# haesungpyun/seoul_tourism_recommendation_NGCF

Measured on AMD Instinct MI355X. Metric: NGCF 3-layer forward: propagated edges/sec + achieved HBM GB/s, d=128, higher is better.
Workload: dtype f32

## Files before the change

include/ngcf_hip.h:

```cpp
#ifndef NGCF_HIP_H
#define NGCF_HIP_H

#include <stdint.h>

#ifdef __cplusplus
extern "C" {
#endif

#define NGCF_OK            0
#define NGCF_ERR_ARG       1
#define NGCF_ERR_HIP       2
#define NGCF_ERR_INDEX     3
#define NGCF_ERR_WORKSPACE 4

typedef struct ngcf_csr ngcf_csr_t;

const char *ngcf_last_error(void);
const char *ngcf_target_arch(void);
#define NGCF_ABI_VERSION 11
int ngcf_version(void);

int ngcf_options_from_env(void);
int ngcf_set_option(const char *name, int64_t value);

int ngcf_prof_enable(int on);
int ngcf_prof_collect(int64_t *n_launches, double *total_ms);

int ngcf_csr_from_coo(const int64_t *rows, const int64_t *cols, const float *vals, int64_t nnz,
                      int64_t n_rows, int64_t n_cols, ngcf_csr_t **out, void *stream);
int ngcf_csr_from_arrays(const int64_t *rowptr, const int32_t *colidx, const float *vals,
                         int64_t n_rows, int64_t n_cols, int64_t nnz, ngcf_csr_t **out, void *stream);
int ngcf_csr_plan(ngcf_csr_t *csr, int32_t seg_len, void *stream);
int ngcf_csr_set_mode(ngcf_csr_t *csr, int mode, void *stream);
int ngcf_csr_filter(const ngcf_csr_t *src, const uint8_t *keep, const int32_t *map, int64_t nnz_kept, ngcf_csr_t **dst,
                    void *stream);
const int32_t *ngcf_csr_filter_pos(const ngcf_csr_t *dst);
int ngcf_csr_filter_remap(const ngcf_csr_t *dst_t, const uint8_t *keep, const int32_t *map, int64_t n_src_entries,
                          const int32_t *pos_l, int32_t *map_out, void *stream);
void ngcf_csr_free(ngcf_csr_t *csr);
int64_t ngcf_csr_nnz(const ngcf_csr_t *csr);
int64_t ngcf_csr_n_rows(const ngcf_csr_t *csr);
int64_t ngcf_csr_n_cols(const ngcf_csr_t *csr);
int64_t ngcf_csr_n_segments(const ngcf_csr_t *csr);
int64_t ngcf_csr_max_row_len(const ngcf_csr_t *csr);
int64_t ngcf_csr_swept_rows(const ngcf_csr_t *csr);
const int64_t *ngcf_csr_rowptr(const ngcf_csr_t *csr);
const int32_t *ngcf_csr_colidx(const ngcf_csr_t *csr);
const float *ngcf_csr_vals(const ngcf_csr_t *csr);

int64_t ngcf_spmm_workspace_bytes(const ngcf_csr_t *csr, int d);
int64_t ngcf_layer_workspace_bytes(const ngcf_csr_t *csr, int d_in, int d_out);

int ngcf_spmm_csr_f32(const ngcf_csr_t *csr, const float *E, int64_t ldE, int d, float *LE,
                      int64_t ldLE, void *workspace, int64_t workspace_bytes, void *stream);

int ngcf_spmm_product_width(const ngcf_csr_t *csr, const float *E, int64_t ldE, int d);

int ngcf_spmm_csr_dropout_f32(const ngcf_csr_t *csr, const float *E, int64_t ldE, int d, float *LE, int64_t ldLE,
                              float drop_p, const uint64_t *seeds, int n_seeds, int transposed,
                              void *workspace, int64_t workspace_bytes, void *stream);

int ngcf_layer_fused_f32(const ngcf_csr_t *csr, const float *E_gather, int64_t ldEg,
                         const float *E_self, int64_t ldEs, int d_in,
                         const float *W1, const float *b1, const float *W2, const float *b2, int d_out,
                         float leaky_slope, float drop_p, uint64_t drop_seed,
                         const float *drop_mask, int64_t ld_mask,
                         float *carry, int64_t ldc, float *norm, int64_t ldn,
                         void *workspace, int64_t workspace_bytes, void *stream);

int64_t ngcf_dense_workspace_bytes(int d_in, int d_out);
int ngcf_layer_dense_f32(const float *LE, int64_t ldLE, const float *E_self, int64_t ldEs,
                         int64_t n_rows, int d_in,
                         const float *W1, const float *b1, const float *W2, const float *b2, int d_out,
                         float leaky_slope, float drop_p, uint64_t drop_seed,
                         const float *drop_mask, int64_t ld_mask,
                         float *carry, int64_t ldc, float *norm, int64_t ldn,
                         void *workspace, int64_t workspace_bytes, void *stream);

// ... 125 lines not shown
```

seoul_tourism_recommendation_ngcf_amd/_lib.py:

```python
from __future__ import annotations

import ctypes as C
import os
import sys

import torch

from . import _build

OK, ERR_ARG, ERR_HIP, ERR_INDEX, ERR_WORKSPACE = 0, 1, 2, 3, 4
ABI_VERSION = 11

_vp, _i64, _i32, _f32, _u64 = C.c_void_p, C.c_int64, C.c_int32, C.c_float, C.c_uint64

PROTOTYPES = {
    "ngcf_last_error": (C.c_char_p, []),
    "ngcf_target_arch": (C.c_char_p, []),
    "ngcf_version": (C.c_int, []),
    "ngcf_options_from_env": (C.c_int, []),
    "ngcf_set_option": (C.c_int, [C.c_char_p, _i64]),
    "ngcf_prof_enable": (C.c_int, [C.c_int]),
    "ngcf_prof_collect": (C.c_int, [C.POINTER(_i64), C.POINTER(C.c_double)]),
    "ngcf_csr_from_coo": (C.c_int, [_vp, _vp, _vp, _i64, _i64, _i64, C.POINTER(_vp), _vp]),
    "ngcf_csr_from_arrays": (C.c_int, [_vp, _vp, _vp, _i64, _i64, _i64, C.POINTER(_vp), _vp]),
    "ngcf_csr_plan": (C.c_int, [_vp, _i32, _vp]),
    "ngcf_csr_set_mode": (C.c_int, [_vp, C.c_int, _vp]),
    "ngcf_csr_filter": (C.c_int, [_vp, _vp, _vp, _i64, C.POINTER(_vp), _vp]),
    "ngcf_csr_filter_pos": (_vp, [_vp]),
    "ngcf_csr_filter_remap": (C.c_int, [_vp, _vp, _vp, _i64, _vp, _vp, _vp]),
    "ngcf_csr_free": (None, [_vp]),
    "ngcf_csr_nnz": (_i64, [_vp]),
    "ngcf_csr_n_rows": (_i64, [_vp]),
    "ngcf_csr_n_cols": (_i64, [_vp]),
    "ngcf_csr_n_segments": (_i64, [_vp]),
    "ngcf_csr_max_row_len": (_i64, [_vp]),
    "ngcf_csr_swept_rows": (_i64, [_vp]),
    "ngcf_csr_rowptr": (_vp, [_vp]),
    "ngcf_csr_colidx": (_vp, [_vp]),
    "ngcf_csr_vals": (_vp, [_vp]),
    "ngcf_spmm_workspace_bytes": (_i64, [_vp, C.c_int]),
    "ngcf_layer_workspace_bytes": (_i64, [_vp, C.c_int, C.c_int]),
    "ngcf_dense_workspace_bytes": (_i64, [C.c_int, C.c_int]),
    "ngcf_spmm_product_width": (C.c_int, [_vp, _vp, _i64, C.c_int]),
    "ngcf_spmm_csr_f32": (C.c_int, [_vp, _vp, _i64, C.c_int, _vp, _i64, _vp, _i64, _vp]),
    "ngcf_spmm_csr_dropout_f32": (C.c_int, [_vp, _vp, _i64, C.c_int, _vp, _i64, _f32, C.POINTER(_u64), C.c_int, C.c_int,
                                            _vp, _i64, _vp]),
    "ngcf_layer_fused_f32": (C.c_int, [_vp, _vp, _i64, _vp, _i64, C.c_int, _vp, _vp, _vp, _vp, C.c_int,
                                       _f32, _f32, _u64, _vp, _i64, _vp, _i64, _vp, _i64, _vp, _i64, _vp]),
    "ngcf_layer_dense_f32": (C.c_int, [_vp, _i64, _vp, _i64, _i64, C.c_int, _vp, _vp, _vp, _vp, C.c_int,
                                       _f32, _f32, _u64, _vp, _i64, _vp, _i64, _vp, _i64, _vp, _i64, _vp]),
    "ngcf_copy_rows_f32": (C.c_int, [_vp, _i64, _vp, _i64, _i64, C.c_int, _vp]),
    "ngcf_copy_rows2_f32": (C.c_int, [_vp, _i64, _vp, _i64, _vp, _i64, _i64, C.c_int, _vp]),
    "ngcf_copy_rows_indexed_f32": (C.c_int, [_vp, _i64, _vp, _i64, _vp, _i64, _i64, C.c_int, _vp]),
    "ngcf_feature_inject_f32": (C.c_int, [_vp, _i64, _i64, C.c_int, C.POINTER(_vp), C.POINTER(_vp),
                                          C.POINTER(_i64), C.c_int, _vp, _i64, C.c_double, _vp, _vp, _vp]),
    "ngcf_seeds_advance": (C.c_int, [_vp, C.c_int, _vp]),
    "ngcf_gather_rows_f32": (C.c_int, [_vp, _i64, C.c_int, _vp, _i64, _i64, _i64, _vp, _i64, _vp, _vp]),
    "ngcf_gather_rows3_f32": (C.c_int, [_vp, _i64, C.c_int] + [_vp, _i64, _i64, _i64, _vp] * 3 + [_i64, _vp, _vp]),
    "ngcf_bpr_workspace_bytes": (_i64, [_i64]),
    "ngcf_bpr_fused_f32": (C.c_int, [_vp, _i64, _vp, _i64, _vp, _i64, C.c_int, _f32, _f32, _vp, _vp, _i64, _vp]),
    "ngcf_bpr_backward_f32": (C.c_int, [_vp, _i64, _vp, _i64, _vp, _i64, C.c_int, _f32, _f32, _vp, _vp, _vp, _vp, _vp]),
    "ngcf_rows_sort_unique": (C.c_int, [_vp, _i64, _i64, _vp, _vp, _vp, _vp, _vp]),
    "ngcf_segment_sum_rows_f32": (C.c_int, [_vp, _i64, C.c_int, _vp, _vp, _i64, _vp, _vp, _vp, _i64, _i64, _vp]),
    "ngcf_layer_bwd_pre_f32": (C.c_int, [_vp, _i64, _vp, _i64, _vp, _i64, _i64, C.c_int, _f32, _f32, _u64, _vp, _i64,
                                         _vp, _vp, _i64, _vp]),
    "ngcf_spmm_t_rows_f32": (C.c_int, [_vp, _vp, _vp, _i64, C.c_int, _vp, _i64, _vp, _i64, _f32, C.POINTER(_u64), C.c_int, _vp, _i64, _vp]),
    "ngcf_layer_bwd_input_workspace_bytes": (_i64, [C.c_int]),
    "ngcf_layer_bwd_input_f32": (C.c_int, [_vp, _i64, _i64, C.c_int, _vp, _vp, C.c_int, _vp, _i64, _vp, _i64, _vp, _i64, _vp, _i64,
                                           _vp, _i64, _vp]),
# ... 105 lines not shown
```

seoul_tourism_recommendation_ngcf_amd/csrc/common.h:

```cpp
#ifndef NGCF_COMMON_H
#define NGCF_COMMON_H

#include <hip/hip_runtime.h>

#include <algorithm>
#include <cstdarg>
#include <cstdint>
#include <cstdio>
#include <cstdlib>
#include <cstring>
#include <numeric>
#include <thread>
#include <vector>

#include "../../include/ngcf_hip.h"

inline thread_local char g_err[512] = "";

inline int fail(int code, const char *fmt, ...)
{
    va_list ap;
    va_start(ap, fmt);
    vsnprintf(g_err, sizeof(g_err), fmt, ap);
    va_end(ap);
// ... 90 lines not shown
    float *vals = nullptr;
    bool owns = false;
    int64_t cap = 0, pos_len = 0;
    int32_t *pos = nullptr;
    int32_t *scan_blk = nullptr;
    bool borrows_plan = false;
    const struct ngcf_csr *filter_src = nullptr;
    int32_t seg_len = 0;
    int64_t n_seg = 0, n_heavy = 0;
    int32_t *seg_row = nullptr;
    int64_t *seg_begin = nullptr;
    int32_t *heavy_row = nullptr;
    int64_t *heavy_seg_ptr = nullptr;
    struct RowGroup {
        int64_t begin, end;
        bool sliceable;
        int32_t col_lo, col_hi;
        bool lds_table = false;
    };
    std::vector<RowGroup> groups;
    int mode = 0;
    struct SegSet {
        int64_t n_seg = 0, n_heavy = 0;
        int32_t *seg_row = nullptr;
        int64_t *seg_begin = nullptr;
        int32_t *heavy_row = nullptr;
        int64_t *heavy_seg_ptr = nullptr;
    };
    struct Swept {
        struct Part {
            int64_t row_lo = 0, row_hi = 0;
            int waves = 0, rows_per_wave = 0;
            int lpe = 16;
            int32_t n_rowpass = 0, n_win = 0, win_cols = 0, col_lo = 0, col_hi = 0;
            int64_t n_slots = 0, n_partial = 0, n_heavy = 0, partial_base = 0;
            int64_t *tptr = nullptr;
            int32_t *e_pack = nullptr;
            float *e_val = nullptr;
            int32_t *dst = nullptr;
            int32_t *prow = nullptr;
            int32_t *heavy_row = nullptr;
            int64_t *heavy_seg_ptr = nullptr;
        };
        std::vector<Part> parts;
        std::vector<char> group_swept;
        SegSet out;
        int64_t n_partial = 0;
        uint32_t *barrier = nullptr;
        mutable hipStream_t barrier_owner[4] = {nullptr, nullptr, nullptr, nullptr};
        mutable int barrier_used = 0;
        int built_mode = 0;
        int lpe = 16;
    } swept;
};


static const int32_t kLdsTableRows = 512;
static const int32_t kDefaultSegLen = 2048;
static inline int32_t default_seg_len(int64_t nnz)
{
    int32_t s = 64;
    while (s < kDefaultSegLen && (int64_t)s * 4096 < nnz) s *= 2;
    return s;
}

void free_swept(ngcf_csr *c);
int build_swept_plan(ngcf_csr *c, hipStream_t stream);
bool swept_usable(const ngcf_csr *c, int64_t ldE, int d);
void prof_mark(hipStream_t stream, int which);

__host__ __device__ inline uint64_t fmix64(uint64_t x)
{
    x ^= x >> 33;
    x *= 0xff51afd7ed558ccdULL;
    x ^= x >> 33;
    x *= 0xc4ceb9fe1a85ec53ULL;
    x ^= x >> 33;
    return x;
}
__device__ inline uint32_t mix32(uint64_t x) { return (uint32_t)fmix64(x); }

__device__ __forceinline__ uint32_t msg_drop_thr(float drop_p)
{
    return drop_p > 0.f ? (uint32_t)((double)drop_p * 4294967296.0) : 0u;
}
// ... 35 lines not shown
    r.s1 = dr.n > 1 ? resolve_seed(dr.seed[1]) : 0;
    r.s2 = dr.n > 2 ? resolve_seed(dr.seed[2]) : 0;
    r.s3 = dr.n > 3 ? resolve_seed(dr.seed[3]) : 0;
    return r;
}

__device__ inline bool edge_keep(const EdgeDropR &dr, int64_t row, int64_t col)
{
    const uint64_t i = (uint64_t)(dr.transposed ? col : row), j = (uint64_t)(dr.transposed ? row : col);
    const uint64_t e = ((i << 32) | (j & 0xffffffffull)) * 0x9E3779B97F4A7C15ULL;
    bool keep = true;
    if (dr.n > 0) keep = mix32(dr.s0 ^ e) >= dr.thr;
    if (dr.n > 1) keep = keep && mix32(dr.s1 ^ e) >= dr.thr;
    if (dr.n > 2) keep = keep && mix32(dr.s2 ^ e) >= dr.thr;
    if (dr.n > 3) keep = keep && mix32(dr.s3 ^ e) >= dr.thr;
    return keep;
}


int spmm_dispatch(const ngcf_csr *c, const float *E, int64_t ldE, int d, float *out, int64_t ldo, void *workspace,
                  int64_t workspace_bytes, hipStream_t stream, const EdgeDrop &dr = EdgeDrop{0, 0, {0, 0, 0, 0}, 0});
int launch_swept(const ngcf_csr *c, const float *E, int64_t ldE, int d, float *out, int64_t ldo, float *partial, int dp,
                 hipStream_t stream, const EdgeDrop &dr);

template <int U> __device__ inline int row_bcast(int x)
{
    return __builtin_amdgcn_update_dpp(0, x, 0x150 + U, 0xf, 0xf, false);
}
template <int U> __device__ inline float row_bcast(float x)
{
    return __int_as_float(__builtin_amdgcn_update_dpp(0, __float_as_int(x), 0x150 + U, 0xf, 0xf, false));
}

template <int VEC> struct VecT;
template <> struct VecT<4> { using type = float4; };
template <> struct VecT<2> { using type = float2; };
template <> struct VecT<1> { using type = float; };

__device__ inline float4 vfma(float s, float4 x, float4 a)
{
    a.x = fmaf(s, x.x, a.x);
    a.y = fmaf(s, x.y, a.y);
    a.z = fmaf(s, x.z, a.z);
    a.w = fmaf(s, x.w, a.w);
    return a;
}
__device__ inline float vfma(float s, float x, float a) { return fmaf(s, x, a); }
__device__ inline float2 vfma(float s, float2 x, float2 a)
{
    a.x = fmaf(s, x.x, a.x);
    a.y = fmaf(s, x.y, a.y);
    return a;
}
__device__ inline float2 vadd(float2 a, float2 b) { return make_float2(a.x + b.x, a.y + b.y); }
__device__ inline float2 vshfl_xor(float2 a, int m)
{
    a.x = __shfl_xor(a.x, m);
    a.y = __shfl_xor(a.y, m);
    return a;
}
__device__ inline float4 vsel(bool p, float4 a, float4 b) { return p ? a : b; }
__device__ inline float vsel(bool p, float a, float b) { return p ? a : b; }
__device__ inline float4 vzero4() { return make_float4(0.f, 0.f, 0.f, 0.f); }
template <int VEC> __device__ inline typename VecT<VEC>::type vzero();
template <> __device__ inline float4 vzero<4>() { return vzero4(); }
template <> __device__ inline float vzero<1>() { return 0.f; }
// ... 40 lines not shown
```

seoul_tourism_recommendation_ngcf_amd/csrc/csr.hip:

```cpp
#include "common.h"

extern "C" const char *ngcf_last_error(void) { return g_err; }
extern "C" const char *ngcf_target_arch(void) { return "gfx950"; }
extern "C" int ngcf_version(void) { return NGCF_ABI_VERSION; }

NgcfOptions g_opts;

namespace {
struct OptField {
    const char *name;
    int NgcfOptions::*i;
    int64_t NgcfOptions::*l;
};
const OptField kOptFields[] = {
    {"no_fork", &NgcfOptions::no_fork, nullptr},
    {"no_slicing", &NgcfOptions::no_slicing, nullptr},
    {"no_ldstab", &NgcfOptions::no_ldstab, nullptr},
    {"no_panel_split", &NgcfOptions::no_panel_split, nullptr},
    {"no_tail_table", &NgcfOptions::no_tail_table, nullptr},
    {"no_pad_product", &NgcfOptions::no_pad_product, nullptr},
    {"fork_min", nullptr, &NgcfOptions::fork_min},
    {"dense_direct", &NgcfOptions::dense_direct, nullptr},
    {"dense_resident", &NgcfOptions::dense_resident, nullptr},
    {"dense_resident_min_rows", &NgcfOptions::dense_resident_min_rows, nullptr},
// ... 72 lines not shown
    c->seg_row = nullptr;
    c->seg_begin = nullptr;
    c->heavy_row = nullptr;
    c->heavy_seg_ptr = nullptr;
    c->n_seg = c->n_heavy = 0;
}

extern "C" void ngcf_csr_free(ngcf_csr_t *c)
{
    if (!c) return;
    free_plan(c);
    free_swept(c);
    if (c->owns) {
        if (c->rowptr) (void)hipFree(c->rowptr);
        if (c->colidx) (void)hipFree(c->colidx);
        if (c->vals) (void)hipFree(c->vals);
    }
    if (c->pos) (void)hipFree(c->pos);
    if (c->scan_blk) (void)hipFree(c->scan_blk);
    delete c;
}

extern "C" int64_t ngcf_csr_nnz(const ngcf_csr_t *c) { return c ? c->nnz : -1; }
extern "C" int64_t ngcf_csr_n_rows(const ngcf_csr_t *c) { return c ? c->n_rows : -1; }
extern "C" int64_t ngcf_csr_n_cols(const ngcf_csr_t *c) { return c ? c->n_cols : -1; }
extern "C" int64_t ngcf_csr_n_segments(const ngcf_csr_t *c) { return c ? c->n_seg : -1; }
extern "C" int64_t ngcf_csr_max_row_len(const ngcf_csr_t *c) { return c ? c->max_row_len : -1; }
extern "C" int64_t ngcf_csr_swept_rows(const ngcf_csr_t *c)
{
    if (!c) return -1;
    int64_t n = 0;
    for (const auto &p : c->swept.parts) n += p.row_hi - p.row_lo;
    return n;
}
extern "C" const int64_t *ngcf_csr_rowptr(const ngcf_csr_t *c) { return c ? c->rowptr : nullptr; }
extern "C" const int32_t *ngcf_csr_colidx(const ngcf_csr_t *c) { return c ? c->colidx : nullptr; }
extern "C" const float *ngcf_csr_vals(const ngcf_csr_t *c) { return c ? c->vals : nullptr; }

__global__ void coo_check_kernel(const int64_t *__restrict__ rows, const int64_t *__restrict__ cols,
                                 int64_t nnz, int64_t n_rows, int64_t n_cols, int32_t *flags)
{
    int64_t i = (int64_t)blockIdx.x * blockDim.x + threadIdx.x;
    const int64_t stride = (int64_t)gridDim.x * blockDim.x;
    bool unsorted = false, bad = false;
    for (; i < nnz; i += stride) {
        const int64_t r = rows[i], c = cols[i];
        bad |= (r < 0) | (r >= n_rows) | (c < 0) | (c >= n_cols);
        if (i + 1 < nnz) unsorted |= rows[i + 1] < r;
    }
    if (unsorted) atomicOr(&flags[0], 1);
    if (bad) atomicOr(&flags[1], 1);
}

__global__ void coo_rowptr_kernel(const int64_t *__restrict__ rows, int64_t nnz, int64_t n_rows,
                                  int64_t *__restrict__ rowptr)
{
    const int64_t r = (int64_t)blockIdx.x * blockDim.x + threadIdx.x;
    if (r > n_rows) return;
    int64_t lo = 0, hi = nnz;
    while (lo < hi) {
        const int64_t mid = (lo + hi) >> 1;
        if (rows[mid] < r)
            lo = mid + 1;
        else
            hi = mid;
    }
// ... 482 lines not shown
```

seoul_tourism_recommendation_ngcf_amd/csrc/spmm_swept.hip:

```cpp
#include "spmm_device.h"

namespace {
constexpr int kLdsBytes = 36 * 16 * 256;
constexpr int kSweptWGs = 256;
constexpr int kRing = 8;
constexpr int kRowBits = 24;
constexpr int kColMask = (1 << kRowBits) - 1;

template <typename F>
void parallel_for(int64_t n, F &&fn, int64_t min_parallel = 64)
{
    unsigned nt = std::thread::hardware_concurrency();
    if (nt > 16) nt = 16;
    if (nt < 1) nt = 1;
    if ((int64_t)nt > n) nt = (unsigned)std::max<int64_t>(n, 1);
    if (n < min_parallel || nt == 1) {
        fn(0, n);
        return;
    }
    std::vector<std::thread> th;
    const int64_t chunk = (n + nt - 1) / nt;
    for (unsigned t = 0; t < nt; ++t) {
        const int64_t lo = t * chunk, hi = std::min<int64_t>(n, lo + chunk);
        if (lo >= hi) break;
// ... 307 lines not shown
            for (int64_t w = 0; w < n_win; ++w) {
                const int64_t b0 = tptr[(size_t)(t * n_win + w)], b1 = tptr[(size_t)(t * n_win + w) + 1];
                if (b0 == b1) continue;
                const int32_t spare = (int32_t)((uint32_t)RW << kRowBits) | (e_pack[(size_t)b0] & kColMask);
                for (int64_t x = b0; x < b1; ++x)
                    if (e_pack[(size_t)x] < 0) e_pack[(size_t)x] = spare;
            }
        }
    });
    std::vector<int32_t> dst((size_t)(n_tasks * RW), -1), prow((size_t)(n_tasks * RW), 0);
    for (size_t i = 0; i < dst.size(); ++i) {
        if (task_piece[i] < 0) continue;
        const int64_t r = pieces[(size_t)task_piece[i]].row;
        dst[i] = r >= 0 ? (int32_t)(row_lo + r) : (int32_t)(-2 - (-1 - r));
        prow[i] = (int32_t)(row_lo + pieces[(size_t)task_piece[i]].src);
    }
    if (ngcf_opts().swept_debug) {
        int64_t mx = 0, mn = INT64_MAX;
        for (int64_t t = 0; t < n_tasks; ++t) {
            const int64_t s = tptr[(size_t)((t + 1) * n_win)] - tptr[(size_t)(t * n_win)];
            mx = std::max(mx, s);
            mn = std::min(mn, s);
        }
        fprintf(stderr, "[swept plan] rows [%lld, %lld) nnz %lld cols [%d, %d]: %d waves x %d rows, %lld row passes, %lld windows x %d "
                        "cols, T %lld, pieces %zu (partial %lld), slots %lld (+%.1f%%), per task %lld..%lld\n",
                (long long)row_lo, (long long)row_hi, (long long)nnz, col_lo, col_hi, waves, RW, (long long)n_rowpass, (long long)n_win,
                win_cols, (long long)T, pieces.size(), (long long)n_partial, (long long)n_slots,
                100.0 * (double)(n_slots - nnz) / (double)nnz, (long long)mn, (long long)mx);
    }
    part.row_lo = row_lo;
    part.row_hi = row_hi;
    part.rows_per_wave = RW;
    part.lpe = LPE;
    part.n_rowpass = (int32_t)n_rowpass;
    part.n_win = (int32_t)n_win;
    part.win_cols = win_cols;
    part.col_lo = col_lo;
    part.col_hi = col_hi;
    part.n_slots = n_slots;
    part.n_partial = n_partial;
    part.n_heavy = (int64_t)heavy_row.size();
    int rc = upload(&part.tptr, tptr, stream);
    if (rc == NGCF_OK) rc = upload(&part.e_pack, e_pack, stream);
    if (rc == NGCF_OK) rc = upload(&part.e_val, e_val, stream);
    if (rc == NGCF_OK) rc = upload(&part.dst, dst, stream);
    if (rc == NGCF_OK) rc = upload(&part.prow, prow, stream);
    if (rc == NGCF_OK && part.n_heavy > 0) rc = upload(&part.heavy_row, heavy_row, stream);
    if (rc == NGCF_OK && part.n_heavy > 0) rc = upload(&part.heavy_seg_ptr, heavy_ptr, stream);
    if (rc == NGCF_OK && hipStreamSynchronize(stream) != hipSuccess) rc = fail(NGCF_ERR_HIP, "swept plan: upload failed");
    if (rc != NGCF_OK) {
        free_part(part);
        return rc;
    }
    part.waves = waves;
    return NGCF_OK;
}
}

void free_swept(ngcf_csr *c)
{
    ngcf_csr::Swept &w = c->swept;
    for (auto &p : w.parts) free_part(p);
    free_segset(w.out);
    if (w.barrier) (void)hipFree(w.barrier);
    w = ngcf_csr::Swept();
}

int build_swept_plan(ngcf_csr *c, hipStream_t stream)
{
    free_swept(c);
    ngcf_csr::Swept &w = c->swept;
    w.built_mode = c->mode;
    w.lpe = ngcf_opts().swept_lpe == 32 ? 32 : 16;
    if (c->mode < 2 || c->n_rows == 0 || c->nnz == 0) return NGCF_OK;
    int dev = 0, cus = 0;
    if (hipGetDevice(&dev) != hipSuccess || hipDeviceGetAttribute(&cus, hipDeviceAttributeMultiprocessorCount, dev) != hipSuccess ||
        cus != kSweptWGs) {
        static bool warned = false;
        if (!warned) {
            warned = true;
            fprintf(stderr, "[ngcf] note: this device reports %d CUs, not %d (an MI355X in SPX mode): the L2-swept SpMM plan is not built and the "
                            "products run on the row-wise kernels (about half the speed on large graphs); ngcf_csr_swept_rows() returns 0\n",
                    cus, kSweptWGs);
        }
        return NGCF_OK;
    }
    w.group_swept.assign(c->groups.size(), 0);
    for (size_t g = 0; g < c->groups.size(); ++g) {
        ngcf_csr::Swept::Part p;
        const int rc = build_part(c, c->groups[g], c->mode == 2, stream, p, w.lpe);
        if (rc != NGCF_OK) {
            free_swept(c);
            return rc;
        }
        if (p.waves == 0) continue;
        w.group_swept[g] = 1;
        w.parts.push_back(p);
    }
    if (w.parts.empty()) return NGCF_OK;
    std::vector<int64_t> rp((size_t)c->n_rows + 1);
    HIP_TRY(hipMemcpyAsync(rp.data(), c->rowptr, sizeof(int64_t) * rp.size(), hipMemcpyDeviceToHost, stream));
    HIP_TRY(hipStreamSynchronize(stream));
    std::vector<int32_t> seg_row, heavy_row;
    std::vector<int64_t> seg_begin, heavy_ptr(1, 0);
    for (size_t g = 0; g < c->groups.size(); ++g) {
        if (w.group_swept[g]) continue;
        for (int64_t r = c->groups[g].begin; r < c->groups[g].end; ++r) {
            if (rp[(size_t)r + 1] - rp[(size_t)r] <= c->seg_len) continue;
            heavy_row.push_back((int32_t)r);
            for (int64_t b = rp[(size_t)r]; b < rp[(size_t)r + 1]; b += c->seg_len) {
                seg_row.push_back((int32_t)r);
                seg_begin.push_back(b);
            }
            heavy_ptr.push_back((int64_t)seg_row.size());
        }
    }
    w.out.n_seg = (int64_t)seg_row.size();
    w.out.n_heavy = (int64_t)heavy_row.size();
    int64_t base = w.out.n_seg;
    for (auto &p : w.parts) {
        p.partial_base = base;
        base += p.n_partial;
        w.n_partial += p.n_partial;
    }
    int rc = NGCF_OK;
    if (w.out.n_seg > 0) {
        rc = upload(&w.out.seg_row, seg_row, stream);
        if (rc == NGCF_OK) rc = upload(&w.out.seg_begin, seg_begin, stream);
        if (rc == NGCF_OK) rc = upload(&w.out.heavy_row, heavy_row, stream);
        if (rc == NGCF_OK) rc = upload(&w.out.heavy_seg_ptr, heavy_ptr, stream);
    }
    if (rc == NGCF_OK && (hipMalloc(&w.barrier, sizeof(uint32_t) * 32 * 8 * 4) != hipSuccess || hipStreamSynchronize(stream) != hipSuccess))
        rc = fail(NGCF_ERR_HIP, "swept plan: allocation failed");
    if (rc != NGCF_OK) free_swept(c);
    return rc;
}

bool swept_usable(const ngcf_csr *c, int64_t ldE, int d)
{
    const ngcf_csr::Swept &w = c->swept;
    if (w.parts.empty() || c->mode < 2 || d % (w.lpe * 4) != 0) return false;
    for (const auto &p : w.parts)
        if (((int64_t)p.col_hi + 1) * ldE * 4 > (int64_t)UINT32_MAX) return false;
    return true;
}

typedef float f32x4 __attribute__((ext_vector_type(4)));
#ifndef NGCF_SWEPT_LABW
#define NGCF_SWEPT_LABW 2
#endif

constexpr int kMaxLaunchParts = 4;
struct SweptPartArgs {
    const int64_t *tptr;
    const int32_t *e_pack;
    const float *e_val;
    const int32_t *dst;
    const int32_t *prow;
    float *partial;
    int n_rowpass, n_win, lead;
};
struct SweptLaunch {
    SweptPartArgs part[kMaxLaunchParts];
    int n_parts;
};

template <int LPE, int RW, int NW, bool DROP>
__global__ __launch_bounds__(NW * 64) void spmm_swept_kernel(SweptLaunch L, int n_slices, const float *__restrict__ E,
                                                             int64_t ldE, float *__restrict__ out, int64_t ldo, int dp, unsigned *bar,
                                                             int max_spin, int sync_k, unsigned prio_cols, int prio_graded,
                                                             EdgeDrop dr_in)
{
    const EdgeDropR dr = resolve_drop(dr_in);
    constexpr int kSW = LPE * 4, kEPR = 64 / LPE, kCH = 16 * kEPR;
    __shared__ float acc_lds[NW * (RW + 1) * kSW];
    __shared__ unsigned wg_cnt[kRing];
    __shared__ int perm_lds;
    __shared__ unsigned xcc_id;
    __shared__ unsigned wg_front;
    const int wave = threadIdx.x >> 6, lane = threadIdx.x & 63;
    const int g = lane / LPE, p = lane % LPE;
    const int held = (lane & 15) * kEPR + g;
    float *wacc = acc_lds + wave * ((RW + 1) * kSW);
    if (threadIdx.x < kRing) wg_cnt[threadIdx.x] = 0;
    if (threadIdx.x == 0) {
        xcc_id = __builtin_amdgcn_s_getreg((3 << 11) | 20) & 7u;
        perm_lds = L.part[0].lead;
        wg_front = 0;
    }
    __syncthreads();
    unsigned *ctr = bar + xcc_id * 32;
    const unsigned members = gridDim.x / 8;
    int perm = L.part[0].lead;
    int step0 = 0;
    const unsigned ld_bytes = (unsigned)ldE * 4u;
    int sweep_no = 0;
    for (int pi = 0; pi < L.n_parts; ++pi) {
    const int64_t *__restrict__ tptr = L.part[pi].tptr;
    const int32_t *__restrict__ e_pack = L.part[pi].e_pack;
    const float *__restrict__ e_val = L.part[pi].e_val;
    const int32_t *__restrict__ dst = L.part[pi].dst;
    float *__restrict__ partial = L.part[pi].partial;
    const int n_rowpass = L.part[pi].n_rowpass, n_win = L.part[pi].n_win, lead = L.part[pi].lead;
    const bool sync = lead >= 0;
    for (int rp = 0; rp < n_rowpass; ++rp) {
        const int64_t task = ((int64_t)rp * gridDim.x + blockIdx.x) * NW + wave;
        const int64_t *tp = tptr + task * n_win;
        const int64_t beg = tp[0], end = tp[n_win];
        int my_row = 0, my_row_hi = 0;
        if (DROP && lane < RW) my_row = L.part[pi].prow[task * RW + lane];
        if (DROP && RW > 64 && lane + 64 < RW) my_row_hi = L.part[pi].prow[task * RW + 64 + lane];
        for (int slice = 0; slice < n_slices; ++slice, ++sweep_no, step0 += (n_win + sync_k - 1) / sync_k) {
            const char *Eb = reinterpret_cast<const char *>(E + slice * kSW);
            for (int i = lane; i < (RW + 1) * kSW; i += 64) wacc[i] = 0.f;
            int b = 0;
// ... 6 lines not shown
                }
            };
            auto cross = [&](int64_t pos, bool crossed) {
                while (b < n_win - 1 && pos >= wend) {
                    if ((b + 1) % sync_k == 0) arrive(step0 + b / sync_k);
                    ++b;
                    wend = wend_next;
                    wend_next = b + 2 <= n_win ? tp[b + 2] : end;
                    crossed = true;
                }
                const int s = step0 + b / sync_k;
                if (crossed && sync && max_spin > 0 && perm < s) {
                    perm = __hip_atomic_load(&perm_lds, __ATOMIC_RELAXED, __HIP_MEMORY_SCOPE_WORKGROUP);
                    int spins = 0;
                    while (perm < s) {
                        const unsigned mine = lane < kRing ? __hip_atomic_load(ctr + lane, __ATOMIC_RELAXED, __HIP_MEMORY_SCOPE_AGENT) : 0u;
                        int t = perm - lead;
                        for (int k = 0; k < kRing - 2 - lead; ++k, ++t) {
                            const unsigned have = __builtin_amdgcn_readlane(mine, t % kRing);
                            if (have < members * (unsigned)(t / kRing + 1)) break;
                        }
                        perm = t + lead;
                        if (perm >= s) break;
                        if (++spins >= max_spin) {
                            max_spin = 0;
                            break;
                        }
                        __builtin_amdgcn_s_sleep(2);
                    }
                    if (lane == 0) atomicMax(&perm_lds, perm);
                }
            };
            const int idle_pk = end > beg ? (RW << kRowBits) | (e_pack[beg] & kColMask) : 0;
            auto load_entries = [&](int64_t pos, int &pk, float &v) {
                const int64_t idx = pos + held;
                const int64_t idc = idx < end ? idx : end - 1;
                const int pk_l = e_pack[idc];
                const float v_l = e_val[idc];
                pk = idx < end ? pk_l : idle_pk;
                v = idx < end ? v_l : 0.f;
                if (DROP) {
                    const int lr = (pk >> kRowBits) & 0x7f;
                    int grow = __shfl(my_row, lr < RW ? lr & 63 : 0);
                    if (RW > 64) {
                        const int hi = __shfl(my_row_hi, lr & 63);
                        grow = lr >= 64 && lr < RW ? hi : grow;
                    }
                    v = edge_keep(dr, grow, pk & kColMask) ? v : 0.f;
                }
            };
            if (end > beg) {
                int pkA, pkB;
                float vA, vB;
                f32x4 xa[8], xb[8];
                unsigned offA;
                const unsigned lane_off = p * 16;
#define NGCF_GATHER(buf, u, j) buf[j] = *reinterpret_cast<const f32x4 *>(Eb + ((unsigned)row_bcast<u>((int)offA) + lane_off));
#define NGCF_GATHER_LO(x) NGCF_GATHER(x, 0, 0) NGCF_GATHER(x, 1, 1) NGCF_GATHER(x, 2, 2) NGCF_GATHER(x, 3, 3) NGCF_GATHER(x, 4, 4) NGCF_GATHER(x, 5, 5) NGCF_GATHER(x, 6, 6) NGCF_GATHER(x, 7, 7)
#define NGCF_GATHER_HI(x) NGCF_GATHER(x, 8, 0) NGCF_GATHER(x, 9, 1) NGCF_GATHER(x, 10, 2) NGCF_GATHER(x, 11, 3) NGCF_GATHER(x, 12, 4) NGCF_GATHER(x, 13, 5) NGCF_GATHER(x, 14, 6) NGCF_GATHER(x, 15, 7)
#define NGCF_ACC(buf, u, j)                                                                        \
    {                                                                                             \
        const int pku = row_bcast<u>(pkA);                                                        \
        const float vu = row_bcast<u>(vA);                                                        \
        if (pku >= 0) {                                                                           \
            f32x4 *a = reinterpret_cast<f32x4 *>(wacc + (pku >> kRowBits) * kSW + p * 4);         \
            f32x4 t = *a;                                                                         \
            t.x = fmaf(vu, buf[j].x, t.x);                                                          \
            t.y = fmaf(vu, buf[j].y, t.y);                                                          \
            t.z = fmaf(vu, buf[j].z, t.z);                                                          \
            t.w = fmaf(vu, buf[j].w, t.w);                                                          \
            *a = t;                                                                               \
        }                                                                                         \
    }
#define NGCF_ACC_LO(x) NGCF_ACC(x, 0, 0) NGCF_ACC(x, 1, 1) NGCF_ACC(x, 2, 2) NGCF_ACC(x, 3, 3) NGCF_ACC(x, 4, 4) NGCF_ACC(x, 5, 5) NGCF_ACC(x, 6, 6) NGCF_ACC(x, 7, 7)
#define NGCF_ACC_HI(x) NGCF_ACC(x, 8, 0) NGCF_ACC(x, 9, 1) NGCF_ACC(x, 10, 2) NGCF_ACC(x, 11, 3) NGCF_ACC(x, 12, 4) NGCF_ACC(x, 13, 5) NGCF_ACC(x, 14, 6) NGCF_ACC(x, 15, 7)
                load_entries(beg, pkA, vA);
                cross(beg, true);
                offA = (unsigned)(pkA & kColMask) * ld_bytes;
                NGCF_GATHER_LO(xa)
                const unsigned sweep_tag = (unsigned)(sweep_no & 0xff) << kRowBits;
                for (int64_t pos = beg; pos < end; pos += kCH) {
                    if (prio_cols) {
                        const unsigned mine = sweep_tag | (unsigned)(__builtin_amdgcn_readfirstlane(pkA) & kColMask);
                        unsigned front = 0;
                        if (lane == 0) front = atomicMax(&wg_front, mine);
                        front = (unsigned)__builtin_amdgcn_readfirstlane((int)front);
                        const unsigned lag = front > mine ? front - mine : 0u;
                        if (prio_graded) {
                            if (lag > 4 * prio_cols) __builtin_amdgcn_s_setprio(3);
                            else if (lag > 2 * prio_cols) __builtin_amdgcn_s_setprio(2);
                            else if (lag > prio_cols) __builtin_amdgcn_s_setprio(1);
                            else __builtin_amdgcn_s_setprio(0);
                        } else {
                            if (lag > prio_cols) __builtin_amdgcn_s_setprio(3);
                            else __builtin_amdgcn_s_setprio(0);
                        }
                    }
                    load_entries(pos + kCH, pkB, vB);
                    if (pos + 8 * kEPR < end) cross(pos + 8 * kEPR, false);
                    NGCF_GATHER_HI(xb)
                    __builtin_amdgcn_s_waitcnt(0xF70 | (NGCF_SWEPT_LABW & 0xf));
                    NGCF_ACC_LO(xa)
                    if (pos + kCH < end) cross(pos + kCH, false);
                    offA = (unsigned)(pkB & kColMask) * ld_bytes;
                    NGCF_GATHER_LO(xa)
                    __builtin_amdgcn_s_waitcnt(0xF70 | (NGCF_SWEPT_LABW & 0xf));
                    NGCF_ACC_HI(xb)
                    pkA = pkB;
                    vA = vB;
                }
#undef NGCF_GATHER
#undef NGCF_GATHER_LO
#undef NGCF_GATHER_HI
#undef NGCF_ACC
#undef NGCF_ACC_LO
#undef NGCF_ACC_HI
            }
            cross(INT64_MAX - 1, false);
            arrive(step0 + (n_win - 1) / sync_k);
            for (int r0 = 0; r0 < RW; r0 += kEPR) {
                const int r = r0 + g;
                if (r < RW) {
                    const int drow = dst[task * RW + r];
                    if (drow != -1) {
                        float *o = drow >= 0 ? out + (int64_t)drow * ldo : partial + (int64_t)(-2 - drow) * dp;
                        *reinterpret_cast<f32x4 *>(o + slice * kSW + p * 4) = *reinterpret_cast<const f32x4 *>(wacc + r * kSW + p * 4);
                    }
                }
            }
        }
    }
    }
}

int launch_swept(const ngcf_csr *c, const float *E, int64_t ldE, int d, float *out, int64_t ldo, float *partial, int dp,
                 hipStream_t stream, const EdgeDrop &dr)
{
    const ngcf_csr::Swept &w = c->swept;
    const NgcfOptions &o = ngcf_opts();
    const int max_spin = o.swept_spin;
    const int lead_env = o.swept_lead;
    const int sync_k = std::max(1, o.swept_sync_every);
    const int kSW = w.lpe * 4;
    const unsigned prio_cols = (unsigned)std::max(0, o.swept_prio_kb) * 1024u / (kSW * 4);
    const int prio_graded = o.swept_prio_graded;
    for (const auto &p : w.parts) {
        SweptLaunch L{};
        const int lead = std::min(lead_env != -2 ? lead_env : (p.n_win >= 8 ? 2 : 1), kRing - 4);
        L.part[L.n_parts++] = SweptPartArgs{p.tptr, p.e_pack, p.e_val, p.dst, p.prow, partial ? partial + p.partial_base * (int64_t)dp : nullptr,
                                            p.n_rowpass, p.n_win, lead};
        int bi = 0;
        for (; bi < w.barrier_used && w.barrier_owner[bi] != stream; ++bi) {}
        if (bi == w.barrier_used) {
            if (w.barrier_used < 4) w.barrier_owner[w.barrier_used++] = stream;
            else bi = 3;
        }
        unsigned *bar_blk = w.barrier + (size_t)bi * 32 * 8;
        HIP_TRY(hipMemsetAsync(bar_blk, 0, sizeof(uint32_t) * 32 * 8, stream));
#define NGCF_SWEPT_LAUNCH(LPE_, RW_, NW_, DROP_)                                                                                    \
    spmm_swept_kernel<LPE_, RW_, NW_, DROP_><<<dim3(kSweptWGs), NW_ * 64, 0, stream>>>(L, d / kSW, E, ldE, out, ldo, dp, bar_blk, \
                                                                                max_spin, sync_k, prio_cols, prio_graded, dr)
        if (w.lpe == 32 && dr.n > 0) NGCF_SWEPT_LAUNCH(32, 18, 16, true);
        else if (w.lpe == 32) NGCF_SWEPT_LAUNCH(32, 18, 16, false);
        else if (dr.n > 0) NGCF_SWEPT_LAUNCH(16, 36, 16, true);
        else NGCF_SWEPT_LAUNCH(16, 36, 16, false);
#undef NGCF_SWEPT_LAUNCH
        LAUNCH_CHECK();
    }
    for (const auto &p : w.parts) {
        if (p.n_heavy == 0) continue;
        spmm_fixup_kernel<4><<<dim3((unsigned)((p.n_heavy + 3) / 4)), 256, 0, stream>>>(
            p.heavy_row, p.heavy_seg_ptr, p.n_heavy, partial + p.partial_base * (int64_t)dp, dp, d, out, ldo);
        LAUNCH_CHECK();
    }
    return NGCF_OK;
}
```

seoul_tourism_recommendation_ngcf_amd/engine.py:

```python
from __future__ import annotations

import ctypes as C
from typing import Optional, Sequence

import torch

from . import _lib

LEAKY_SLOPE = 0.2


def _require_device(t: torch.Tensor, what: str):
    if not t.is_cuda:
        raise RuntimeError(
            f"{what} is on '{t.device}': the NGCF propagation engine runs on a ROCm device only "
            "(hand-written HIP kernels, no CPU/PyTorch fallback). Move the module and inputs to 'cuda'.")


def _f32c(t: torch.Tensor, what: str) -> torch.Tensor:
    _require_device(t, what)
    if t.dtype != torch.float32:
        raise RuntimeError(f"{what}: expected float32, got {t.dtype}")
    return t

# ... 100 lines not shown
        if keep.dtype not in (torch.uint8, torch.bool) or not keep.is_contiguous():
            raise RuntimeError("filtered: keep must be a contiguous uint8 / bool tensor")
        if entry_map is not None and (entry_map.dtype != torch.int32 or not entry_map.is_contiguous() or entry_map.numel() != self.nnz):
            raise RuntimeError("filtered: entry_map must be a contiguous int32 tensor with one element per stored entry")
        if entry_map is None and keep.numel() != self.nnz:
            raise RuntimeError(f"filtered: {keep.numel()} keep flags for {self.nnz} stored entries")
        out = C.c_void_p(reuse._h.value if reuse is not None and reuse._h.value else None)
        with _on(keep.device):
            rc = lib.ngcf_csr_filter(self._h, _ptr(keep), _ptr(entry_map), int(nnz_kept), C.byref(out), _stream())
        if reuse is not None:
            reuse._h = C.c_void_p(0 if rc == _lib.OK else (out.value or 0))
        _lib.check(rc)
        res = LaplacianCSR(out.value, keep_alive=(self,))
        res.src_nnz = self.nnz
        return res

    @property
    def filter_pos(self) -> int:
        return int(_lib.load().ngcf_csr_filter_pos(self._h) or 0)

    def plan(self, seg_len: int):
        _lib.check(_lib.load().ngcf_csr_plan(self._h, int(seg_len), _stream()))

    def set_mode(self, mode: int):
        _lib.check(_lib.load().ngcf_csr_set_mode(self._h, int(mode), _stream()))

    @property
    def n_segments(self) -> int:
        return int(_lib.load().ngcf_csr_n_segments(self._h))

    @property
    def swept_rows(self) -> int:
        return int(_lib.load().ngcf_csr_swept_rows(self._h))

    def layer_workspace_bytes(self, d_in: int, d_out: int) -> int:
        n = int(_lib.load().ngcf_layer_workspace_bytes(self._h, d_in, d_out))
        if n < 0:
            raise RuntimeError(f"unsupported layer widths d_in={d_in} d_out={d_out} (1..512)")
        return n

    def spmm_workspace_bytes(self, d: int) -> int:
        return int(_lib.load().ngcf_spmm_workspace_bytes(self._h, d))

    def close(self):
        if getattr(self, "_h", None) is not None and self._h.value:
            _lib.load().ngcf_csr_free(self._h)
            self._h = C.c_void_p(0)

    def __del__(self):
        try:
            self.close()
        except Exception:
            pass


class Workspace:

    def __init__(self):
        self.buf: Optional[torch.Tensor] = None

    def get(self, nbytes: int, device) -> torch.Tensor:
        if self.buf is None or self.buf.numel() < nbytes or self.buf.device != torch.device(device):
            self.buf = torch.empty(max(int(nbytes), 256), dtype=torch.uint8, device=device)
        return self.buf


# ... 698 lines not shown
```

Baseline: 28.20 billion.

## Add per-part LPE=8 swept SpMM variant for large row groups

```diff
diff --git a/include/ngcf_hip.h b/include/ngcf_hip.h
--- a/include/ngcf_hip.h
+++ b/include/ngcf_hip.h
@@ -44,6 +44,8 @@
 int64_t ngcf_csr_n_segments(const ngcf_csr_t *csr);
 int64_t ngcf_csr_max_row_len(const ngcf_csr_t *csr);
 int64_t ngcf_csr_swept_rows(const ngcf_csr_t *csr);
+int ngcf_csr_swept_parts(const ngcf_csr_t *csr);
+int ngcf_csr_swept_part_info(const ngcf_csr_t *csr, int part, int64_t *info);
 const int64_t *ngcf_csr_rowptr(const ngcf_csr_t *csr);
 const int32_t *ngcf_csr_colidx(const ngcf_csr_t *csr);
 const float *ngcf_csr_vals(const ngcf_csr_t *csr);
diff --git a/seoul_tourism_recommendation_ngcf_amd/_lib.py b/seoul_tourism_recommendation_ngcf_amd/_lib.py
--- a/seoul_tourism_recommendation_ngcf_amd/_lib.py
+++ b/seoul_tourism_recommendation_ngcf_amd/_lib.py
@@ -35,6 +35,8 @@
     "ngcf_csr_n_segments": (_i64, [_vp]),
     "ngcf_csr_max_row_len": (_i64, [_vp]),
     "ngcf_csr_swept_rows": (_i64, [_vp]),
+    "ngcf_csr_swept_parts": (C.c_int, [_vp]),
+    "ngcf_csr_swept_part_info": (C.c_int, [_vp, C.c_int, _vp]),
     "ngcf_csr_rowptr": (_vp, [_vp]),
     "ngcf_csr_colidx": (_vp, [_vp]),
     "ngcf_csr_vals": (_vp, [_vp]),
diff --git a/seoul_tourism_recommendation_ngcf_amd/csrc/common.h b/seoul_tourism_recommendation_ngcf_amd/csrc/common.h
--- a/seoul_tourism_recommendation_ngcf_amd/csrc/common.h
+++ b/seoul_tourism_recommendation_ngcf_amd/csrc/common.h
@@ -146,6 +146,7 @@
             int64_t row_lo = 0, row_hi = 0;
             int waves = 0, rows_per_wave = 0;
             int lpe = 16;
+            int64_t nnz = 0;
             int32_t n_rowpass = 0, n_win = 0, win_cols = 0, col_lo = 0, col_hi = 0;
             int64_t n_slots = 0, n_partial = 0, n_heavy = 0, partial_base = 0;
             int64_t *tptr = nullptr;
@@ -164,7 +165,6 @@
         mutable hipStream_t barrier_owner[4] = {nullptr, nullptr, nullptr, nullptr};
         mutable int barrier_used = 0;
         int built_mode = 0;
-        int lpe = 16;
     } swept;
 };
 
@@ -266,6 +266,12 @@
     return __int_as_float(__builtin_amdgcn_update_dpp(0, __float_as_int(x), 0x150 + U, 0xf, 0xf, false));
 }
 
+template <int U> __device__ inline int row_bcast_halves(int x0, int x1)
+{
+    const int lo = __builtin_amdgcn_update_dpp(0, x0, 0x150 + U, 0xf, 0x3, false);
+    return __builtin_amdgcn_update_dpp(lo, x1, 0x150 + U, 0xf, 0xc, false);
+}
+
 template <int VEC> struct VecT;
 template <> struct VecT<4> { using type = float4; };
 template <> struct VecT<2> { using type = float2; };
diff --git a/seoul_tourism_recommendation_ngcf_amd/csrc/csr.hip b/seoul_tourism_recommendation_ngcf_amd/csrc/csr.hip
--- a/seoul_tourism_recommendation_ngcf_amd/csrc/csr.hip
+++ b/seoul_tourism_recommendation_ngcf_amd/csrc/csr.hip
@@ -128,6 +128,15 @@
     int64_t n = 0;
     for (const auto &p : c->swept.parts) n += p.row_hi - p.row_lo;
     return n;
+}
+extern "C" int ngcf_csr_swept_parts(const ngcf_csr_t *c) { return c ? (int)c->swept.parts.size() : -1; }
+extern "C" int ngcf_csr_swept_part_info(const ngcf_csr_t *c, int part, int64_t *info)
+{
+    if (!c || !info || part < 0 || part >= (int)c->swept.parts.size()) return fail(NGCF_ERR_ARG, "ngcf_csr_swept_part_info: bad argument");
+    const auto &p = c->swept.parts[(size_t)part];
+    const int64_t v[8] = {p.row_lo, p.row_hi, p.lpe, p.n_rowpass, p.n_win, p.win_cols, p.nnz, p.n_slots};
+    for (int i = 0; i < 8; ++i) info[i] = v[i];
+    return NGCF_OK;
 }
 extern "C" const int64_t *ngcf_csr_rowptr(const ngcf_csr_t *c) { return c ? c->rowptr : nullptr; }
 extern "C" const int32_t *ngcf_csr_colidx(const ngcf_csr_t *c) { return c ? c->colidx : nullptr; }
diff --git a/seoul_tourism_recommendation_ngcf_amd/csrc/spmm_swept.hip b/seoul_tourism_recommendation_ngcf_amd/csrc/spmm_swept.hip
--- a/seoul_tourism_recommendation_ngcf_amd/csrc/spmm_swept.hip
+++ b/seoul_tourism_recommendation_ngcf_amd/csrc/spmm_swept.hip
@@ -363,6 +363,7 @@
     part.row_hi = row_hi;
     part.rows_per_wave = RW;
     part.lpe = LPE;
+    part.nnz = nnz;
     part.n_rowpass = (int32_t)n_rowpass;
     part.n_win = (int32_t)n_win;
     part.win_cols = win_cols;
@@ -402,7 +403,6 @@
     free_swept(c);
     ngcf_csr::Swept &w = c->swept;
     w.built_mode = c->mode;
-    w.lpe = ngcf_opts().swept_lpe == 32 ? 32 : 16;
     if (c->mode < 2 || c->n_rows == 0 || c->nnz == 0) return NGCF_OK;
     int dev = 0, cus = 0;
     if (hipGetDevice(&dev) != hipSuccess || hipDeviceGetAttribute(&cus, hipDeviceAttributeMultiprocessorCount, dev) != hipSuccess ||
@@ -419,7 +419,10 @@
     w.group_swept.assign(c->groups.size(), 0);
     for (size_t g = 0; g < c->groups.size(); ++g) {
         ngcf_csr::Swept::Part p;
-        const int rc = build_part(c, c->groups[g], c->mode == 2, stream, p, w.lpe);
+        const int forced = ngcf_opts().swept_lpe;
+        const int64_t cap16 = (int64_t)kSweptWGs * (kLdsBytes / 256);
+        const int lpe = forced == 8 || forced == 16 || forced == 32 ? forced : (c->groups[g].end - c->groups[g].begin > cap16 ? 8 : 16);
+        const int rc = build_part(c, c->groups[g], c->mode == 2, stream, p, lpe);
         if (rc != NGCF_OK) {
             free_swept(c);
             return rc;
@@ -470,9 +473,9 @@
 bool swept_usable(const ngcf_csr *c, int64_t ldE, int d)
 {
     const ngcf_csr::Swept &w = c->swept;
-    if (w.parts.empty() || c->mode < 2 || d % (w.lpe * 4) != 0) return false;
+    if (w.parts.empty() || c->mode < 2) return false;
     for (const auto &p : w.parts)
-        if (((int64_t)p.col_hi + 1) * ldE * 4 > (int64_t)UINT32_MAX) return false;
+        if (d % (p.lpe * 4) != 0 || ((int64_t)p.col_hi + 1) * ldE * 4 > (int64_t)UINT32_MAX) return false;
     return true;
 }
 
@@ -480,6 +483,14 @@
 #ifndef NGCF_SWEPT_LABW
 #define NGCF_SWEPT_LABW 2
 #endif
+template <int LPE> constexpr int kSweptLabW = NGCF_SWEPT_LABW;
+template <> constexpr int kSweptLabW<8> = 2;
+
+template <int LPE, int U> __device__ inline int ent_bcast(int x0, int x1) { return LPE == 8 ? row_bcast_halves<U>(x0, x1) : row_bcast<U>(x0); }
+template <int LPE, int U> __device__ inline float ent_bcast(float x0, float x1)
+{
+    return __int_as_float(ent_bcast<LPE, U>(__float_as_int(x0), __float_as_int(x1)));
+}
 
 constexpr int kMaxLaunchParts = 4;
 struct SweptPartArgs {
@@ -511,7 +522,8 @@
     __shared__ unsigned wg_front;
     const int wave = threadIdx.x >> 6, lane = threadIdx.x & 63;
     const int g = lane / LPE, p = lane % LPE;
-    const int held = (lane & 15) * kEPR + g;
+    constexpr bool kTwo = LPE == 8;
+    const int held = (lane & 15) * kEPR + (kTwo ? (lane >> 4) * 2 : g);
     float *wacc = acc_lds + wave * ((RW + 1) * kSW);
     if (threadIdx.x < kRing) wg_cnt[threadIdx.x] = 0;
     if (threadIdx.x == 0) {
@@ -584,36 +596,49 @@
                 }
             };
             const int idle_pk = end > beg ? (RW << kRowBits) | (e_pack[beg] & kColMask) : 0;
-            auto load_entries = [&](int64_t pos, int &pk, float &v) {
+            auto drop_entry = [&](int pk, float &v) {
+                const int lr = (pk >> kRowBits) & 0x7f;
+                int grow = __shfl(my_row, lr < RW ? lr & 63 : 0);
+                if (RW > 64) {
+                    const int hi = __shfl(my_row_hi, lr & 63);
+                    grow = lr >= 64 && lr < RW ? hi : grow;
+                }
+                v = edge_keep(dr, grow, pk & kColMask) ? v : 0.f;
+            };
+            auto load_entries = [&](int64_t pos, int &pk, int &pk1, float &v, float &v1) {
                 const int64_t idx = pos + held;
-                const int64_t idc = idx < end ? idx : end - 1;
-                const int pk_l = e_pack[idc];
-                const float v_l = e_val[idc];
-                pk = idx < end ? pk_l : idle_pk;
-                v = idx < end ? v_l : 0.f;
+                const int64_t idc = idx < end ? idx : end - (kTwo ? 2 : 1);
+                if (kTwo) {
+                    const int2 pk_l = *reinterpret_cast<const int2 *>(e_pack + idc);
+                    const float2 v_l = *reinterpret_cast<const float2 *>(e_val + idc);
+                    pk = idx < end ? pk_l.x : idle_pk;
+                    pk1 = idx < end ? pk_l.y : idle_pk;
+                    v = idx < end ? v_l.x : 0.f;
+                    v1 = idx < end ? v_l.y : 0.f;
+                } else {
+                    const int pk_l = e_pack[idc];
+                    const float v_l = e_val[idc];
+                    pk = pk1 = idx < end ? pk_l : idle_pk;
+                    v = v1 = idx < end ? v_l : 0.f;
+                }
                 if (DROP) {
-                    const int lr = (pk >> kRowBits) & 0x7f;
-                    int grow = __shfl(my_row, lr < RW ? lr & 63 : 0);
-                    if (RW > 64) {
-                        const int hi = __shfl(my_row_hi, lr & 63);
-                        grow = lr >= 64 && lr < RW ? hi : grow;
-                    }
-                    v = edge_keep(dr, grow, pk & kColMask) ? v : 0.f;
+                    drop_entry(pk, v);
+                    if (kTwo) drop_entry(pk1, v1);
                 }
             };
             if (end > beg) {
-                int pkA, pkB;
-                float vA, vB;
+                int pkA, pkB, pkA1, pkB1;
+                float vA, vB, vA1, vB1;
                 f32x4 xa[8], xb[8];
-                unsigned offA;
+                unsigned offA, offA1;
                 const unsigned lane_off = p * 16;
-#define NGCF_GATHER(buf, u, j) buf[j] = *reinterpret_cast<const f32x4 *>(Eb + ((unsigned)row_bcast<u>((int)offA) + lane_off));
+#define NGCF_GATHER(buf, u, j) buf[j] = *reinterpret_cast<const f32x4 *>(Eb + ((unsigned)ent_bcast<LPE, u>((int)offA, (int)offA1) + lane_off));
 #define NGCF_GATHER_LO(x) NGCF_GATHER(x, 0, 0) NGCF_GATHER(x, 1, 1) NGCF_GATHER(x, 2, 2) NGCF_GATHER(x, 3, 3) NGCF_GATHER(x, 4, 4) NGCF_GATHER(x, 5, 5) NGCF_GATHER(x, 6, 6) NGCF_GATHER(x, 7, 7)
 #define NGCF_GATHER_HI(x) NGCF_GATHER(x, 8, 0) NGCF_GATHER(x, 9, 1) NGCF_GATHER(x, 10, 2) NGCF_GATHER(x, 11, 3) NGCF_GATHER(x, 12, 4) NGCF_GATHER(x, 13, 5) NGCF_GATHER(x, 14, 6) NGCF_GATHER(x, 15, 7)
 #define NGCF_ACC(buf, u, j)                                                                        \
     {                                                                                             \
-        const int pku = row_bcast<u>(pkA);                                                        \
-        const float vu = row_bcast<u>(vA);                                                        \
+        const int pku = ent_bcast<LPE, u>(pkA, pkA1);                                             \
+        const float vu = ent_bcast<LPE, u>(vA, vA1);                                              \
         if (pku >= 0) {                                                                           \
             f32x4 *a = reinterpret_cast<f32x4 *>(wacc + (pku >> kRowBits) * kSW + p * 4);         \
             f32x4 t = *a;                                                                         \
@@ -626,9 +651,10 @@
     }
 #define NGCF_ACC_LO(x) NGCF_ACC(x, 0, 0) NGCF_ACC(x, 1, 1) NGCF_ACC(x, 2, 2) NGCF_ACC(x, 3, 3) NGCF_ACC(x, 4, 4) NGCF_ACC(x, 5, 5) NGCF_ACC(x, 6, 6) NGCF_ACC(x, 7, 7)
 #define NGCF_ACC_HI(x) NGCF_ACC(x, 8, 0) NGCF_ACC(x, 9, 1) NGCF_ACC(x, 10, 2) NGCF_ACC(x, 11, 3) NGCF_ACC(x, 12, 4) NGCF_ACC(x, 13, 5) NGCF_ACC(x, 14, 6) NGCF_ACC(x, 15, 7)
-                load_entries(beg, pkA, vA);
+                load_entries(beg, pkA, pkA1, vA, vA1);
                 cross(beg, true);
                 offA = (unsigned)(pkA & kColMask) * ld_bytes;
+                offA1 = (unsigned)(pkA1 & kColMask) * ld_bytes;
                 NGCF_GATHER_LO(xa)
                 const unsigned sweep_tag = (unsigned)(sweep_no & 0xff) << kRowBits;
                 for (int64_t pos = beg; pos < end; pos += kCH) {
@@ -648,18 +674,21 @@
                             else __builtin_amdgcn_s_setprio(0);
                         }
                     }
-                    load_entries(pos + kCH, pkB, vB);
+                    load_entries(pos + kCH, pkB, pkB1, vB, vB1);
                     if (pos + 8 * kEPR < end) cross(pos + 8 * kEPR, false);
                     NGCF_GATHER_HI(xb)
-                    __builtin_amdgcn_s_waitcnt(0xF70 | (NGCF_SWEPT_LABW & 0xf));
+                    __builtin_amdgcn_s_waitcnt(0xF70 | (kSweptLabW<LPE> & 0xf));
                     NGCF_ACC_LO(xa)
                     if (pos + kCH < end) cross(pos + kCH, false);
                     offA = (unsigned)(pkB & kColMask) * ld_bytes;
+                    offA1 = (unsigned)(pkB1 & kColMask) * ld_bytes;
                     NGCF_GATHER_LO(xa)
-                    __builtin_amdgcn_s_waitcnt(0xF70 | (NGCF_SWEPT_LABW & 0xf));
+                    __builtin_amdgcn_s_waitcnt(0xF70 | (kSweptLabW<LPE> & 0xf));
                     NGCF_ACC_HI(xb)
                     pkA = pkB;
+                    pkA1 = pkB1;
                     vA = vB;
+                    vA1 = vB1;
                 }
 #undef NGCF_GATHER
 #undef NGCF_GATHER_LO
@@ -693,11 +722,12 @@
     const int max_spin = o.swept_spin;
     const int lead_env = o.swept_lead;
     const int sync_k = std::max(1, o.swept_sync_every);
-    const int kSW = w.lpe * 4;
-    const unsigned prio_cols = (unsigned)std::max(0, o.swept_prio_kb) * 1024u / (kSW * 4);
+    const unsigned prio_bytes = (unsigned)std::max(0, o.swept_prio_kb) * 1024u;
     const int prio_graded = o.swept_prio_graded;
     for (const auto &p : w.parts) {
         SweptLaunch L{};
+        const int kSW = p.lpe * 4;
+        const unsigned prio_cols = prio_bytes / (kSW * 4);
         const int lead = std::min(lead_env != -2 ? lead_env : (p.n_win >= 8 ? 2 : 1), kRing - 4);
         L.part[L.n_parts++] = SweptPartArgs{p.tptr, p.e_pack, p.e_val, p.dst, p.prow, partial ? partial + p.partial_base * (int64_t)dp : nullptr,
                                             p.n_rowpass, p.n_win, lead};
@@ -712,8 +742,10 @@
 #define NGCF_SWEPT_LAUNCH(LPE_, RW_, NW_, DROP_)                                                                                    \
     spmm_swept_kernel<LPE_, RW_, NW_, DROP_><<<dim3(kSweptWGs), NW_ * 64, 0, stream>>>(L, d / kSW, E, ldE, out, ldo, dp, bar_blk, \
                                                                                 max_spin, sync_k, prio_cols, prio_graded, dr)
-        if (w.lpe == 32 && dr.n > 0) NGCF_SWEPT_LAUNCH(32, 18, 16, true);
-        else if (w.lpe == 32) NGCF_SWEPT_LAUNCH(32, 18, 16, false);
+        if (p.lpe == 32 && dr.n > 0) NGCF_SWEPT_LAUNCH(32, 18, 16, true);
+        else if (p.lpe == 32) NGCF_SWEPT_LAUNCH(32, 18, 16, false);
+        else if (p.lpe == 8 && dr.n > 0) NGCF_SWEPT_LAUNCH(8, 72, 16, true);
+        else if (p.lpe == 8) NGCF_SWEPT_LAUNCH(8, 72, 16, false);
         else if (dr.n > 0) NGCF_SWEPT_LAUNCH(16, 36, 16, true);
         else NGCF_SWEPT_LAUNCH(16, 36, 16, false);
 #undef NGCF_SWEPT_LAUNCH
diff --git a/seoul_tourism_recommendation_ngcf_amd/engine.py b/seoul_tourism_recommendation_ngcf_amd/engine.py
--- a/seoul_tourism_recommendation_ngcf_amd/engine.py
+++ b/seoul_tourism_recommendation_ngcf_amd/engine.py
@@ -156,6 +156,17 @@
     @property
     def swept_rows(self) -> int:
         return int(_lib.load().ngcf_csr_swept_rows(self._h))
+
+    @property
+    def swept_parts(self) -> list:
+        import ctypes
+        lib, parts = _lib.load(), []
+        for i in range(int(lib.ngcf_csr_swept_parts(self._h))):
+            v = (ctypes.c_int64 * 8)()
+            _lib.check(lib.ngcf_csr_swept_part_info(self._h, i, v))
+            parts.append({"row_lo": v[0], "row_hi": v[1], "lpe": v[2], "n_rowpass": v[3], "n_win": v[4], "win_cols": v[5],
+                          "nnz": v[6], "n_slots": v[7], "padding": (v[7] - v[6]) / max(v[6], 1)})
+        return parts
 
     def layer_workspace_bytes(self, d_in: int, d_out: int) -> int:
         n = int(_lib.load().ngcf_layer_workspace_bytes(self._h, d_in, d_out))
```

Result: slower. 27.43 billion (-2.7%).
